# Plachtaa/VALL-E-X

Hardware: AMD Instinct MI355X
Metric: audio-seconds/sec (AR+NAR+Vocos end to end; AR codec-tokens/sec in ar_tokens_per_s), batch32 8s utt (higher is better)
Workload: dtype f32 (cached AR decode step) + f16x2 (operands split into fp16 head + tail = 22 significant bits, tail x tail dropped, fp32 accumulate) for the prefill / NAR projections and full-sequence attention

## Files before the change

vall-e-x_amd/_build.py:

```python
from __future__ import annotations

import os
import subprocess
import sys
from concurrent.futures import ThreadPoolExecutor

HERE = os.path.dirname(os.path.abspath(__file__))
CSRC = os.path.join(HERE, "csrc")
LIB = os.path.join(CSRC, "libvallex_hip.so")
PREFLIGHT = os.path.join(CSRC, "vx_preflight.bin")
SOURCES = ["gemm_f32.hip", "gemm_f16x2.hip", "gemm_bf16x3.hip", "gemm_bf16x3_dma.hip", "rows.hip", "attn_full.hip", "attn_full_x3.hip", "attn_full_h2.hip", "decode.hip", "beams.hip", "admit.hip", "serve.hip", "serve_sample.hip", "vocos.hip", "encodec.hip", "engine.hip", "weights.hip", "vocoders.hip", "bench_harness.hip"]
HEADERS = ["vx_common.h"]
ENGINE_TUS = ("engine.hip", "beams.hip", "admit.hip", "serve.hip", "serve_sample.hip", "weights.hip", "vocoders.hip", "bench_harness.hip")
ENGINE_HEADERS = ["engine_ctx.h", os.path.join("..", "..", "include", "vallex_hip.h"),
                  os.path.join("..", "..", "include", "vallex_hip_dev.h")]
FLAGS = ["--offload-arch=gfx950", "-O3", "-std=c++17", "-fPIC", "-Wall", "-Wno-unused-result",
         "-mllvm", "-amdgpu-kernarg-preload-count=16"]


def _hipcc() -> str:
    for cand in (os.environ.get("HIPCC"), "/opt/rocm/bin/hipcc", "hipcc"):
        if cand and (os.path.sep not in cand or os.path.exists(cand)):
            return cand
    return "hipcc"


def _digest(paths, extra=()) -> str:
    import hashlib
    h = hashlib.sha256()
# ... 91 lines not shown
```

vall-e-x_amd/csrc/engine.hip:

```cpp
#include "engine_ctx.h"

#include <deque>
#include <memory>

namespace {
thread_local std::string g_create_err;
}

namespace vxe {

const float* W(vx_ctx* c, const std::string& name) {
  auto it = c->w.find(name);
  return it == c->w.end() ? nullptr : it->second.d;
}

static int ring_slot(vx_ctx* c, size_t n, char** slot) {
  PinRing& r = c->ring;
  if (!r.base) FAIL(VX_ESTATE, "the context has no pinned transfer ring");
  const size_t a = (n + 255) & ~(size_t)255;
  if (r.head + a > r.cap) if (int e = xfer_sync(c)) return e;
  *slot = r.base + r.head;
  r.head += a;
  return VX_OK;
}
// ... 424 lines not shown
  a.uniforms_stride = c->cur_batch;
  a.seed_dev = c->seed_dev;
  a.force_eos_at = s ? s->force_eos_at : -1;
  a.commit = commit;
  a.cur_tok = c->cur_tok; a.cur_pos = c->cur_pos; a.ctx_len = c->ctx_len; a.n_gen = c->n_gen; a.active = c->active;
  a.n_active = c->n_active; a.slot_meta = c->slot_meta; a.slot_of = c->slot_of;
  a.text_len = c->text_len; a.gen = c->gen; a.gen_stride = c->gen_stride; a.logits_out = logits_out;
  a.sum_logp = (s && s->best_of > 1) ? c->sum_logp : nullptr;
  a.batch = c->cur_batch;
  if (commit) {
    a.emb_tab = W(c, "ar_audio_embedding.word_embeddings.weight"); a.emb_alpha = W(c, "ar_audio_position.alpha");
    a.pe = c->pe; a.ln_g = c->ar[0].n1_w; a.ln_b = c->ar[0].n1_b; a.emb_h = c->dh; a.emb_xp = c->xp;
    a.wt = c->sb_chain ? 0 : 1;
  }
  return a;
}

void ar_step_launches(vx_ctx* c, const SampleArgs* sa, const ServeSampleArgs* rsa) {
  const int nb = c->cur_batch, NL = c->NL;
  hipStream_t st = c->stream;
  const size_t cache_layer = (size_t)c->mbr * N_HEAD * c->Tmax * D_HEAD;
  if (!sa && !rsa)
    launch_dec_embed_ln_pack(c->cur_tok, c->cur_pos, W(c, "ar_audio_embedding.word_embeddings.weight"),
                             W(c, "ar_audio_position.alpha"), c->pe, c->dh, c->ar[0].n1_w, c->ar[0].n1_b, c->xp, nb, st);
  if (c->sb_chain) {
    float *hr = c->dh, *hw = c->dh2;
    for (int l = 0; l < NL; ++l) {
      const LayerW& L = c->ar[l];
      if (c->sb_qkv) {
        {
// ... 24 lines not shown
      { ProfScope ps(c, 1); LAUNCH(launch_skinny_gemm_sb_combine(L.out_wp, c->p_o, D_MODEL, SK_OUT, c->part_o, c->part_ml, c->nsplit, nb, st)); }
      }
      {
        ProfScope ps(c, 1);
        LAUNCH(launch_skinny16_sb_ln(L.l1_wp, L.l1_b, c->xp4, D_FF, c->p_o, SK_OUT, L.out_b, hr, hw, L.n2_w, L.n2_b, nb, st));
        std::swap(hr, hw);
      }
      { ProfScope ps(c, 1); launch_skinny_gemm(L.l2_wp, c->xp4, c->p_o, D_MODEL, D_FF, SK_L2, st); }
    }
    {
      ProfScope ps(c, 1);
      LAUNCH(launch_skinny_gemm_sb_ln(c->pred_wp, c->p_logits, PRED_NPAD, SK_PRED, c->p_o, SK_L2, c->ar[NL - 1].l2_b, hr, nullptr,
                               W(c, "ar_decoder.norm.weight"), W(c, "ar_decoder.norm.bias"), nb, st));
    }
    if (rsa) LAUNCH(launch_serve_sample(*rsa, st));
    else if (sa) LAUNCH(launch_dec_sample(*sa, st));
    return;
  }
  for (int l = 0; l < NL; ++l) {
    const LayerW& L = c->ar[l];
    {
      ProfScope ps(c, 1);
      if (c->qkv_bal) launch_skinny_qkv_balanced(L.in_wp, c->xp, c->p_qkv, st);
      else launch_skinny_gemm(L.in_wp, c->xp, c->p_qkv, 3 * D_MODEL, D_MODEL, SK_QKV, st, true);
    }
    const bool fused = c->fuse_out && (c->nsplit == 1 || c->split_fused);
    {
      ProfScope ps(c, 0);
      LAUNCH(launch_dec_attn(c->p_qkv, c->qkv_bal ? SK_QKV_BALANCED : SK_QKV, L.in_b, c->kc + l * cache_layer, c->vc + l * cache_layer, c->Tmax, c->slot_meta,
                      c->xp_att, c->part_o, c->part_ml, c->nsplit, nb, fused ? L.out_wh : nullptr, c->p_oh, st));
    }
// ... 2 lines not shown
    } else if (fused) {
      launch_dec_reduce_ln_pack(c->p_oh, N_HEAD, D_MODEL, L.out_b, c->dh, c->dh, L.n2_w, L.n2_b, c->xp, nb, st);
    } else {
      if (c->nsplit > 1) launch_dec_attn_combine(c->part_o, c->part_ml, c->nsplit, c->active, c->xp_att, nb, st);
      { ProfScope ps(c, 1); launch_skinny_gemm(L.out_wp, c->xp_att, c->p_o, D_MODEL, D_MODEL, SK_OUT, st, true); }
      launch_dec_reduce_ln_pack(c->p_o, SK_OUT, D_MODEL, L.out_b, c->dh, c->dh, L.n2_w, L.n2_b, c->xp, nb, st);
    }
    { ProfScope ps(c, 1); launch_skinny16_relu_pack(L.l1_wp, c->xp, L.l1_b, c->xp4, D_FF, D_MODEL, st); }
    { ProfScope ps(c, 1); launch_skinny_gemm(L.l2_wp, c->xp4, c->p_o, D_MODEL, D_FF, SK_L2, st, true); }
    const float* ng = (l + 1 < NL) ? c->ar[l + 1].n1_w : W(c, "ar_decoder.norm.weight");
    const float* nbp = (l + 1 < NL) ? c->ar[l + 1].n1_b : W(c, "ar_decoder.norm.bias");
    launch_dec_reduce_ln_pack(c->p_o, SK_L2, D_MODEL, L.l2_b, c->dh, c->dh, ng, nbp, c->xp, nb, st);
  }
  { ProfScope ps(c, 1); launch_skinny_gemm(c->pred_wp, c->xp, c->p_logits, PRED_NPAD, D_MODEL, SK_PRED, st, true); }
  if (rsa) LAUNCH(launch_serve_sample(*rsa, st));
  else if (sa) LAUNCH(launch_dec_sample(*sa, st));
}

static_assert(SK_QKV == 4, "dec_attn_kernel<*, 4> sums four QKV slabs in its prologue");
static_assert(SK_OUT == 4, "skinny16_sb_kernel<4> / dec_reduce_ln_pack<4> are the instantiated out_proj consumers");
static_assert(SK_L2 == 8 || SK_L2 == 4, "skinny_gemm_sb_kernel<0, 8 | 4> are the instantiated linear2 consumers");
static_assert(SK_PRED == 4 || SK_PRED == 2 || SK_PRED == 1, "dec_sample_kernel<4 | 2 | 1>");

int launch_status(vx_ctx* c) {
  if (!c->launch_fail) return VX_OK;
  const char* what = c->launch_fail;
  c->launch_fail = nullptr;
  FAIL(VX_EINVAL, "kernel configuration not compiled into this library: %s", what);
}

constexpr int GRAPH_STEPS = 4;
// ... 49 lines not shown
    const long steps = std::min<long>(s->uniforms_steps, c->gen_stride + 1);
    if (steps * nb > c->uniforms_cap) FAIL(VX_EINVAL, "too many uniforms (%ld steps)", steps);
    std::vector<float> u((size_t)steps * nb);
    for (long t = 0; t < steps; ++t)
      for (int i = 0; i < nb; ++i) u[t * nb + i] = s->uniforms[t * ub + (long)r0 * beams + i];
    H2D(c->d_uniforms, u.data(), u.size() * sizeof(float));
    SYNC();
  }
  H2D(c->seed_dev, &seed, sizeof seed);
  SampleArgs sa = make_sample_args(c, s, 1, nullptr);
  std::vector<int> act(nb);
  bool any = true, raised = false;
  auto first_sample = [&]() -> int {
    int flag = 0;
    HIPCHK(hipMemsetAsync(c->sum_logp, 0, MB * sizeof(float), c->stream));
    LAUNCH(launch_dec_sample(sa, c->stream));
    if (int e = launch_status(c)) return e;
    D2H(act.data(), c->active, nb * sizeof(int));
    if (range_guarded(c) && !direct_f32) D2H(&flag, c->range_flag, sizeof(int));
    SYNC();
    raised = flag != 0;
    any = std::any_of(act.begin(), act.end(), [](int v) { return v != 0; });
    return VX_OK;
  };
  if (int e = first_sample()) return e;
  if (!direct_f32) fb_outcome(c, raised, c->fb_prefill_raises, c->sticky_prefill_f32, c->sticky_prefill_age);
  if (raised) {
    HIPCHK(hipMemsetAsync(c->range_flag, 0, sizeof(int), c->stream));
    ++c->st_fb_prefill; ++c->fb_total;
    if (int e = ensure_f32_buffers(c)) return e;
    {
      F32Scope f32(c);
      if (int e = ar_prefill(c, b, r0, nb_rows, beams)) return e;
      if (int e = first_sample()) return e;
    }
  }
  char sig[160];
  snprintf(sig, sizeof sig, "b%d ns%d c%d%d%d k%d t%a u%d f%d l%d", nb, c->nsplit, (int)c->sb_chain, (int)c->sb_qkv, (int)c->split_fused, sa.top_k, sa.temperature,
           sa.uniforms != nullptr, sa.force_eos_at, sa.sum_logp != nullptr);
  const int sync_every = s->sync_every > 0 ? s->sync_every : 8;
  const int hard_cap = s->force_eos_at >= 0 ? std::min(c->gen_stride + 2, s->force_eos_at) : c->gen_stride + 2;
  int steps = 0;
  const int gs = (c->graph_multi && sync_every % GRAPH_STEPS == 0) ? GRAPH_STEPS : 1;
  while (any && steps < hard_cap) {
    const int n = (steps % gs == 0 && steps + gs <= hard_cap) ? gs : 1;
    if (int e = ar_step_run(c, &sa, sig, n)) return e;
    steps += n;
    if (steps % sync_every == 0) {
      D2H(act.data(), c->active, nb * sizeof(int));
      SYNC();
      any = std::any_of(act.begin(), act.end(), [](int v) { return v != 0; });
    }
  }
  n_gen.resize(nb);
// ... 234 lines not shown
    adm[drow[i]] = 1;
  }
  const long o_tab = mb.add(tab), o_adm = mb.add(adm), o_saved = mb.add(saved);
  UniformCols uc;
  if (int e = uniform_cols(c, b, s, drow, crow, mb, uc)) return e;
  if (int e = upload_meta(c)) return e;
  uniform_cols_launch(c, s, uc, mb);
  if (int e = prefill_layers(c, p, mb)) return e;
  launch_admit_rows(mb.dev(o_tab), k, prefill_hsrc(c, p), c->dh2, c->cur_tok, c->cur_pos, c->ctx_len, c->n_gen, c->text_len,
                    c->slot_meta, c->slot_of, c->stream);
  launch_dec_reduce_ln_pack(nullptr, 0, D_MODEL, nullptr, c->dh2, nullptr, W(c, "ar_decoder.norm.weight"),
                            W(c, "ar_decoder.norm.bias"), c->xp_att, nd, c->stream);
  launch_skinny_gemm(c->pred_wp, c->xp_att, c->p_logits, PRED_NPAD, D_MODEL, SK_PRED, c->stream);
  int* sv = c->imeta + o_saved;
  launch_admit_mask(0, mb.dev(o_adm), sv, nd, c->active, c->slot_meta, c->slot_of, c->n_active, c->stream);
  LAUNCH(launch_dec_sample(sa, c->stream));
  launch_admit_mask(1, mb.dev(o_adm), sv, nd, c->active, c->slot_meta, c->slot_of, c->n_active, c->stream);
  return launch_status(c);
}

int infer_continuous(vx_ctx* c, const vx_batch* b, const vx_sampling* s, vx_row_done_fn on_row, void* user, int64_t* out_codes,
                     int32_t out_stride, int32_t* out_lens) {
  const int B = b->batch, nd = std::min(c->mbr, B);
  hipEvent_t e0 = c->ev_t[0], e1 = c->ev_t[1], e2 = c->ev_t[2];
  HIPCHK(hipEventRecord(e0, c->stream));
  std::vector<int> occ(nd, -1), done_by(nd, 0), act(nd, 0), ng(nd, 0), slot_of(nd);
  std::vector<std::vector<int>> rowgen(B);
  std::vector<int> pend;
  int next = 0;
  long steps = 0;
  const int first_cap = s->force_eos_at >= 0 ? std::min(c->gen_stride, s->force_eos_at) : c->gen_stride;
// ... 3 lines not shown
  };
  SampleArgs sa{};
  auto round = [&](const std::vector<int>& drow, const std::vector<int>& crow) -> int {
    const bool first = occ[0] < 0 && next == 0;
    bool raised = false;
    auto attempt = [&](bool read_flag) -> int {
      if (first) {
        if (int e = ar_prefill(c, b, 0, nd)) return e;
        sa = make_sample_args(c, s, 1, nullptr);
        sa.uniforms = c->d_uniforms;
        MetaBuilder mb(c);
        UniformCols uc;
        if (int e = uniform_cols(c, b, s, drow, crow, mb, uc)) return e;
        if (int e = upload_meta(c)) return e;
        uniform_cols_launch(c, s, uc, mb);
        LAUNCH(launch_dec_sample(sa, c->stream));
        if (int e = launch_status(c)) return e;
        D2H(slot_of.data(), c->slot_of, nd * sizeof(int));
      } else if (int e = admit_rows(c, b, s, sa, drow, crow, slot_of)) return e;
      int flag = 0;
      D2H(act.data(), c->active, nd * sizeof(int));
      D2H(ng.data(), c->n_gen, nd * sizeof(int));
      if (read_flag) D2H(&flag, c->range_flag, sizeof(int));
      SYNC();
      raised = flag != 0;
      return VX_OK;
    };
    const bool direct_f32 = fb_direct(c, c->sticky_prefill_f32, c->sticky_prefill_age);
    if (direct_f32) {
      ++c->st_fb_prefill; ++c->fb_total;
      if (int e = ensure_f32_buffers(c)) return e;
// ... 42 lines not shown
        o[0] = codes0[(size_t)i * c->gen_stride + t];
        for (int st = 0; st < N_Q - 1; ++st) o[st + 1] = oc[(size_t)st * sumT + off + t];
      }
      off += T[i];
      if (on_row) on_row(user, r, o0, T[i]);
    }
    return VX_OK;
  };

  {
    std::vector<int> first(nd);
    for (int i = 0; i < nd; ++i) first[i] = i;
    if (int e = round(first, first)) return e;
  }
  char sig[160];
  snprintf(sig, sizeof sig, "b%d ns%d c%d%d%d k%d t%a u%d f%d l%d", nd, c->nsplit, (int)c->sb_chain, (int)c->sb_qkv, (int)c->split_fused, sa.top_k,
           sa.temperature, sa.uniforms != nullptr, sa.force_eos_at, sa.sum_logp != nullptr);
  const int sync_every = s->sync_every > 0 ? s->sync_every : 8;
  const int gs = (c->graph_multi && sync_every % GRAPH_STEPS == 0) ? GRAPH_STEPS : 1;
  for (;;) {
    std::vector<int> freed;
    for (int d = 0; d < nd; ++d) {
      if (occ[d] < 0 || act[d]) continue;
      const int r = occ[d];
      if (ng[d] > out_stride) FAIL(VX_EINVAL, "out_stride %d too small for %d frames", out_stride, ng[d]);
      rowgen[r].assign(ng[d], 0);
      if (ng[d]) D2H(rowgen[r].data(), c->gen + (size_t)d * c->gen_stride, ng[d] * sizeof(int));
      pend.push_back(r);
      occ[d] = -1;
    }
    for (int d = 0; d < nd; ++d) if (occ[d] < 0) freed.push_back(d);
    if (next < B && !freed.empty()) {
// ... 704 lines not shown
  for (int d = 0; d < v->nd; ++d) v->slot_of[d] = d;
  if (!c->row_smp) {
    if (int e = dev_alloc(c, &c->row_smp, 4 * MB)) { delete v; return e; }
  }
  if (int e = serve_setup(c, v->nd)) { delete v; return e; }
  const SampleArgs sa = make_sample_args(c, &v->s, 1, nullptr);
  ServeSampleArgs& r = v->rsa;
  r.partial = sa.partial; r.splitk = sa.splitk; r.npad = sa.npad;
  r.row_smp = c->row_smp;
  r.uniforms = c->d_uniforms; r.uniforms_stride = sa.uniforms_stride;
  r.cur_tok = sa.cur_tok; r.cur_pos = sa.cur_pos; r.ctx_len = sa.ctx_len; r.n_gen = sa.n_gen; r.active = sa.active;
  r.n_active = sa.n_active; r.text_len = sa.text_len; r.slot_meta = sa.slot_meta; r.slot_of = sa.slot_of;
  r.gen = sa.gen; r.gen_stride = sa.gen_stride; r.sum_logp = c->sum_logp; r.batch = sa.batch;
  r.emb_tab = sa.emb_tab; r.emb_alpha = sa.emb_alpha; r.pe = sa.pe; r.ln_g = sa.ln_g; r.ln_b = sa.ln_b; r.emb_h = sa.emb_h;
  r.emb_xp = sa.emb_xp; r.wt = sa.wt;
  char sig[160];
  snprintf(sig, sizeof sig, "b%d ns%d c%d%d%d serve-rows u1 l1", v->nd, c->nsplit, (int)c->sb_chain, (int)c->sb_qkv, (int)c->split_fused);
  v->sig = sig;
  c->serve = v;
  *out = v;
  return VX_OK;
}

int vx_serve_submit(vx_serve* v, const vx_batch* b, const vx_request* req, int64_t* ids_out) {
  if (!v || !req) return VX_EINVAL;
  return serve_submit(v, b, req, nullptr, ids_out);
}

int vx_serve_submit_ex(vx_serve* v, const vx_batch* b, const vx_request* req, const vx_request_sampling* smp, int64_t* ids_out) {
  if (!v || !req) return VX_EINVAL;
  return serve_submit(v, b, req, smp, ids_out);
}
// ... 102 lines not shown
```

vall-e-x_amd/csrc/engine_ctx.h:

```cpp
#pragma once

#include <math.h>
#include <stdio.h>
#include <stdlib.h>
#include <string.h>

#include <algorithm>
#include <array>
#include <map>
#include <string>
#include <thread>
#include <vector>

#include "../../include/vallex_hip.h"
#include "vx_common.h"

using namespace vx;

namespace vxe {

struct Tensor {
  float* d = nullptr;
  std::vector<int64_t> shape;
  size_t n = 0;
// ... 69 lines not shown
  unsigned short* fa3 = nullptr;
  unsigned short* pred_w3[N_Q - 1] = {};
  float *fx = nullptr, *fxn = nullptr, *fqkv = nullptr, *fatt = nullptr, *fffn = nullptr, *fyemb = nullptr,
        *flogits = nullptr;
  int* imeta = nullptr;
  long imeta_cap = 0;
  std::vector<int> hmeta;

  float *kc = nullptr, *vc = nullptr;
  float *dh = nullptr, *dh2 = nullptr, *xp = nullptr, *xp_att = nullptr, *xp4 = nullptr;
  bool sb_qkv = false;
  int sb_qkv_rows = 4, sb_qkv_nsplit = 0;
  bool sb_chain = false;
  bool sb_fuse = true;
  bool qkv_bal = true;
  float* qk_new = nullptr;
  float *p_qkv = nullptr, *p_o = nullptr, *p_oh = nullptr, *p_logits = nullptr, *part_o = nullptr, *part_ml = nullptr;
  std::map<const unsigned short*, int> w_shift;
  bool nar_trim = true;
  bool balance_rows = true;
  bool fuse_out = true;
  int fuse_split = 1;
  bool split_fused = false;
  float *d_logits = nullptr, *d_uniforms = nullptr, *sum_logp = nullptr;
  long uniforms_cap = 0;
  int *cur_tok = nullptr, *cur_pos = nullptr, *ctx_len = nullptr, *n_gen = nullptr, *active = nullptr,
      *text_len = nullptr, *gen = nullptr, *force_tok = nullptr, *n_active = nullptr, *slot_meta = nullptr, *slot_of = nullptr;
  int gen_stride = 0;
  int cur_batch = 0;
  int nsplit = 1;
// ... 153 lines not shown
                           int* row_smp, hipStream_t s);
void launch_serve_cancel(unsigned rows, int nrows, int* active, int* slot_meta, const int* slot_of, int* n_active, hipStream_t s);

struct ServeSampleArgs {
  const float* partial; int splitk; int npad;
  const int* row_smp;
  const float* uniforms; int uniforms_stride;
  int* cur_tok; int* cur_pos; int* ctx_len; int* n_gen; int* active; int* n_active; const int* text_len;
  int* slot_meta; const int* slot_of;
  int* gen; int gen_stride;
  float* sum_logp;
  int batch;
  const float* emb_tab; const float* emb_alpha; const float* pe; const float* ln_g; const float* ln_b;
  float* emb_h; float* emb_xp;
  int wt;
};
bool launch_serve_sample(const ServeSampleArgs& a, hipStream_t s);

struct F32Scope {
  vx_ctx* c;
  int gm;
  bool ax;
  explicit F32Scope(vx_ctx* c_) : c(c_), gm(c_->gemm_mode), ax(c_->attn_x3) { c->gemm_mode = 2; c->attn_x3 = false; }
  ~F32Scope() { c->gemm_mode = gm; c->attn_x3 = ax; }
};

}
```

vall-e-x_amd/csrc/serve_sample.hip:

```cpp
#include "engine_ctx.h"

namespace vxe {
namespace {

constexpr int SPL = 17;

__device__ __forceinline__ void store_wt(float* p, const f32x4& v, bool wt) {
  if (wt) asm volatile("global_store_dwordx4 %0, %1, off sc1" :: "v"(p), "v"(v) : "memory");
  else *reinterpret_cast<f32x4*>(p) = v;
}

__device__ __forceinline__ float sum64f(float v) {
  int x = __builtin_bit_cast(int, v);
  v += __builtin_bit_cast(float, __builtin_amdgcn_update_dpp(0, x, 0xB1, 0xF, 0xF, true));
  x = __builtin_bit_cast(int, v);
  v += __builtin_bit_cast(float, __builtin_amdgcn_update_dpp(0, x, 0x4E, 0xF, 0xF, true));
  x = __builtin_bit_cast(int, v);
  v += __builtin_bit_cast(float, __builtin_amdgcn_update_dpp(0, x, 0x141, 0xF, 0xF, true));
  x = __builtin_bit_cast(int, v);
  v += __builtin_bit_cast(float, __builtin_amdgcn_update_dpp(0, x, 0x140, 0xF, 0xF, true));
  x = __builtin_bit_cast(int, v);
  v += __builtin_bit_cast(float, __builtin_amdgcn_update_dpp(0, x, 0x142, 0xA, 0xF, false));
  x = __builtin_bit_cast(int, v);
  v += __builtin_bit_cast(float, __builtin_amdgcn_update_dpp(0, x, 0x143, 0xC, 0xF, false));
// ... 45 lines not shown
    for (int e = 0; e < 4; ++e) { const float d = v[i][e] - mean; q += d * d; }
  const float rstd = 1.0f / sqrtf(sum64f(q) * (1.0f / D_MODEL) + LN_EPS);
#pragma unroll
  for (int i = 0; i < 4; ++i) {
    const int c4 = lane + 64 * i;
    f32x4 o;
#pragma unroll
    for (int e = 0; e < 4; ++e) o[e] = (v[i][e] - mean) * rstd * gg[i][e] + be[i][e];
    store_wt(xp + (((long)(c4 >> 1) * 64) + b + 32 * (c4 & 1)) * 4, o, wt);
  }
}

template <int SK>
__global__ __launch_bounds__(64) void serve_sample_kernel(ServeSampleArgs a) {
  __shared__ float lg[64 * SPL];
  const int b = blockIdx.x, lane = threadIdx.x;
  if (a.active[b] == 0) return;
  const int ngen = a.n_gen[b], pos = a.cur_pos[b], ctx = a.ctx_len[b], tlen = a.text_len[b], slot = a.slot_of[b];
  const int4 smp = *reinterpret_cast<const int4*>(a.row_smp + 4 * b);
  const int top_k = smp.x, force_eos_at = smp.z;
  const float temperature = __builtin_bit_cast(float, smp.y);
  {
    float pp[SPL][SK];
#pragma unroll
    for (int i = 0; i < SPL; ++i) {
      const int n = lane + 64 * i, nc = n < AR_LOGITS ? n : AR_LOGITS - 1;
#pragma unroll
      for (int ks = 0; ks < SK; ++ks) pp[i][ks] = a.partial[((long)ks * MB + b) * a.npad + nc];
    }
#pragma unroll
    for (int i = 0; i < SPL; ++i) {
      const int n = lane + 64 * i;
      float t = pp[i][0];
      if (SK == 2) t = t + pp[i][1];
      if (SK == 4) t = ((t + pp[i][1]) + pp[i][2]) + pp[i][3];
      if (n >= AR_LOGITS) t = -INFINITY;
      lg[n] = t;
    }
  }
  __syncthreads();

  const float u = a.uniforms[(long)ngen * a.uniforms_stride + b];
  f32x4 pe4[4], gg[4], be[4];
  float alpha = 0.f;
// ... 3 lines not shown
    for (int i = 0; i < 4; ++i) {
      const int c = (lane + 64 * i) * 4;
      pe4[i] = *reinterpret_cast<const f32x4*>(a.pe + (long)(pos + 1) * D_MODEL + c);
      gg[i] = *reinterpret_cast<const f32x4*>(a.ln_g + c);
      be[i] = *reinterpret_cast<const f32x4*>(a.ln_b + c);
    }
  }

  float v[SPL];
#pragma unroll
  for (int j = 0; j < SPL; ++j) v[j] = lg[lane * SPL + j];
  if (temperature != 1.0f) {
#pragma unroll
    for (int j = 0; j < SPL; ++j) v[j] = v[j] / temperature;
  }
  float mx = -INFINITY;
#pragma unroll
  for (int j = 0; j < SPL; ++j) mx = fmaxf(mx, v[j]);
  mx = max64f(mx);

  if (top_k > 0 && top_k < AR_LOGITS) {
    float thr = mx;
    for (int it = 1; it < top_k && thr != -INFINITY; ++it) {
      float cur = -INFINITY;
#pragma unroll
      for (int j = 0; j < SPL; ++j) if (v[j] < thr) cur = fmaxf(cur, v[j]);
      thr = max64f(cur);
    }
    int cnt = 0;
#pragma unroll
    for (int j = 0; j < SPL; ++j) cnt += (v[j] >= thr);
    if (sum64i(cnt) != top_k) {
      float prev = INFINITY;
      int count = 0;
      thr = mx;
      while (true) {
        float cur = -INFINITY;
#pragma unroll
        for (int j = 0; j < SPL; ++j) if (v[j] < prev) cur = fmaxf(cur, v[j]);
        cur = max64f(cur);
        int c2 = 0;
#pragma unroll
        for (int j = 0; j < SPL; ++j) c2 += (v[j] == cur);
        count += sum64i(c2);
        thr = cur;
        if (count >= top_k || cur == -INFINITY) break;
        prev = cur;
      }
    }
#pragma unroll
    for (int j = 0; j < SPL; ++j) if (v[j] < thr) v[j] = -INFINITY;
  }
  float e[SPL], loc = 0.f;
#pragma unroll
  for (int j = 0; j < SPL; ++j) { e[j] = expf(v[j] - mx); loc += e[j]; }
  float incl = loc;
#pragma unroll
  for (int o = 1; o < 64; o <<= 1) {
    const float t = __shfl_up(incl, o, 64);
    if (lane >= o) incl += t;
  }
  const float total = __builtin_bit_cast(float, __builtin_amdgcn_readlane(__builtin_bit_cast(int, incl), 63));
  const float thresh = u * total;
  float c = incl - loc;
  int cand = 0x7fffffff, lastnz = -1;
#pragma unroll
  for (int j = 0; j < SPL; ++j) {
    if (e[j] > 0.f) {
      c += e[j];
      lastnz = lane * SPL + j;
      if (c > thresh && cand == 0x7fffffff) cand = lane * SPL + j;
    }
  }
  cand = minmax64i<false>(cand);
  const int last_all = minmax64i<true>(lastnz);
  int tok = cand == 0x7fffffff ? last_all : cand;
  if ((unsigned)tok > (unsigned)EOS_ID) tok = EOS_ID;

  if (tok / SPL == lane) {
    float vt = 0.f;
#pragma unroll
    for (int j = 0; j < SPL; ++j) if (tok - lane * SPL == j) vt = v[j];
    a.sum_logp[b] += (vt - mx) - logf(total);
  }

  if (force_eos_at >= 0 && ngen >= force_eos_at) tok = EOS_ID;
  const bool stop = tok == EOS_ID || (1 + ngen) > 16 * tlen || ngen >= a.gen_stride;
  if (lane == 0) {
    if (stop) {
      a.active[b] = 0;
// ... 36 lines not shown
```

vall-e-x_amd/csrc/weights.hip:

```cpp
#include "engine_ctx.h"

namespace {

int need(vx_ctx* c, const std::string& name, std::initializer_list<int64_t> shape) {
  auto it = c->w.find(name);
  if (it == c->w.end()) FAIL(VX_ENOTFOUND, "missing tensor '%s'", name.c_str());
  if (it->second.shape != std::vector<int64_t>(shape)) FAIL(VX_EINVAL, "tensor '%s' has the wrong shape", name.c_str());
  return VX_OK;
}

int pack(vx_ctx* c, const float* Wt, int N, int K, int Npad, float** out) {
  if (int e = dev_alloc(c, out, (size_t)Npad * K, false)) return e;
  launch_pack_weight(Wt, N, K, *out, Npad, c->stream);
  return VX_OK;
}

}

extern "C" {

int vx_load_tensor(vx_ctx* c, const char* name, const float* data, const int64_t* shape, int32_t ndim) {
  if (!c) return VX_EINVAL;
  if (!name || !data || !shape || ndim < 0 || ndim > 4) FAIL(VX_EINVAL, "bad tensor argument");
  if (c->finalized) FAIL(VX_ESTATE, "weights already finalized");
// ... 96 lines not shown
  if (range_guarded(c) && (e = ensure_f32_buffers(c))) return e;
  if ((e = dev_alloc(c, &c->fyemb, (size_t)M * d))) return e;
  if ((e = dev_alloc(c, &c->flogits, (size_t)((long)c->mbr * c->cfg.max_new + 128) * AUDIO_VOCAB))) return e;
  c->imeta_cap = std::max(M * 24, (long)c->cfg.max_batch * c->cfg.max_new * 12) + 65536;
  if ((e = dev_alloc(c, &c->imeta, (size_t)c->imeta_cap))) return e;
  const size_t cache = (size_t)NL * c->mbr * N_HEAD * c->Tmax * D_HEAD;
  if ((e = dev_alloc(c, &c->kc, cache, true))) return e;
  if ((e = dev_alloc(c, &c->vc, cache, true))) return e;
  if ((e = dev_alloc(c, &c->dh, (size_t)MB * d))) return e;
  if ((e = dev_alloc(c, &c->dh2, (size_t)MB * d))) return e;
  if (const char* ev = getenv("VX_SB_FUSE")) c->sb_fuse = !(ev[0] == '0');
  if ((e = dev_alloc(c, &c->xp, (size_t)MB * d))) return e;
  if ((e = dev_alloc(c, &c->xp_att, (size_t)MB * d))) return e;
  if ((e = dev_alloc(c, &c->xp4, (size_t)2 * MB * f))) return e;
  if (const char* ev = getenv("VX_QKV_BALANCED")) c->qkv_bal = !(ev[0] == '0');
  static_assert(SK_QKV_BAL_Q == 8 && SK_QKV_BAL_KV == SK_QKV, "skinny_qkv_bal_kernel writes 8 q slabs and SK_QKV k / v slabs into p_qkv");
  if ((e = dev_alloc(c, &c->p_qkv, (size_t)std::max(SK_QKV, SK_QKV_BAL_Q) * MB * 3 * d))) return e;
  if ((e = dev_alloc(c, &c->p_o, (size_t)std::max(SK_OUT, SK_L2) * MB * d))) return e;
  if ((e = dev_alloc(c, &c->p_oh, (size_t)4 * N_HEAD * MB * d))) return e;
  if (const char* ev = getenv("VX_FUSE_OUT")) c->fuse_out = !(ev[0] == '0');
  if (c->Tmax < DEC_ATTN_TILE) c->fuse_out = false;
  if (const char* ev = getenv("VX_BALANCE_ROWS")) c->balance_rows = !(ev[0] == '0');
  if (const char* ev = getenv("VX_NAR_TRIM")) c->nar_trim = ev[0] == '1';
  if (const char* ev = getenv("VX_GRAPH_MULTI")) c->graph_multi = !(ev[0] == '0');
  if (const char* ev = getenv("VX_SB_QKV")) c->sb_qkv_rows = atoi(ev);
  if (const char* ev = getenv("VX_SB_QKV_NSPLIT")) c->sb_qkv_nsplit = atoi(ev);
  if (const char* ev = getenv("VX_FUSE_SPLIT")) c->fuse_split = atoi(ev);
  if (const char* ev = getenv("VX_ATT_NSPLIT")) c->att_nsplit_force = std::max(0, std::min(16, atoi(ev)));
  if ((e = dev_alloc(c, &c->p_logits, (size_t)SK_PRED * MB * PRED_NPAD))) return e;
  if ((e = dev_alloc(c, &c->part_o, (size_t)MB * N_HEAD * 16 * D_HEAD))) return e;
// ... 392 lines not shown
```

Baseline: 378.4.

## Add fast single-pass top-k selection for AR sampling kernels

Adds a new sampling kernel and a shared selection header. It finds the top-k candidates in one pass, using a per-lane-max threshold plus ballot compaction into LDS, instead of the iterative max-below-threshold loop that costs one wave reduction per k. It also uses DPP for the prefix scan and skips the last-nonzero reduction unless it is needed. The decode, serve and admit paths route to this kernel by default, and the old loop stays as a fallback when more than 64 candidates or ties are present. Tie-breaking and floating-point equivalence are risks, and the extra LDS use could change occupancy.

Result: no change. 380.5 (median of 6 runs) (+0.6%).

```diff
diff --git a/vall-e-x_amd/_build.py b/vall-e-x_amd/_build.py
--- a/vall-e-x_amd/_build.py
+++ b/vall-e-x_amd/_build.py
@@ -9,10 +9,10 @@
 CSRC = os.path.join(HERE, "csrc")
 LIB = os.path.join(CSRC, "libvallex_hip.so")
 PREFLIGHT = os.path.join(CSRC, "vx_preflight.bin")
-SOURCES = ["gemm_f32.hip", "gemm_f16x2.hip", "gemm_bf16x3.hip", "gemm_bf16x3_dma.hip", "rows.hip", "attn_full.hip", "attn_full_x3.hip", "attn_full_h2.hip", "decode.hip", "beams.hip", "admit.hip", "serve.hip", "serve_sample.hip", "vocos.hip", "encodec.hip", "engine.hip", "weights.hip", "vocoders.hip", "bench_harness.hip"]
+SOURCES = ["gemm_f32.hip", "gemm_f16x2.hip", "gemm_bf16x3.hip", "gemm_bf16x3_dma.hip", "rows.hip", "attn_full.hip", "attn_full_x3.hip", "attn_full_h2.hip", "decode.hip", "beams.hip", "admit.hip", "serve.hip", "serve_sample.hip", "sample_fast.hip", "vocos.hip", "encodec.hip", "engine.hip", "weights.hip", "vocoders.hip", "bench_harness.hip"]
 HEADERS = ["vx_common.h"]
-ENGINE_TUS = ("engine.hip", "beams.hip", "admit.hip", "serve.hip", "serve_sample.hip", "weights.hip", "vocoders.hip", "bench_harness.hip")
-ENGINE_HEADERS = ["engine_ctx.h", os.path.join("..", "..", "include", "vallex_hip.h"),
+ENGINE_TUS = ("engine.hip", "beams.hip", "admit.hip", "serve.hip", "serve_sample.hip", "sample_fast.hip", "weights.hip", "vocoders.hip", "bench_harness.hip")
+ENGINE_HEADERS = ["engine_ctx.h", "sample_select.h", os.path.join("..", "..", "include", "vallex_hip.h"),
                   os.path.join("..", "..", "include", "vallex_hip_dev.h")]
 FLAGS = ["--offload-arch=gfx950", "-O3", "-std=c++17", "-fPIC", "-Wall", "-Wno-unused-result",
          "-mllvm", "-amdgpu-kernarg-preload-count=16"]
diff --git a/vall-e-x_amd/csrc/engine.hip b/vall-e-x_amd/csrc/engine.hip
--- a/vall-e-x_amd/csrc/engine.hip
+++ b/vall-e-x_amd/csrc/engine.hip
@@ -462,6 +462,13 @@
     a.wt = c->sb_chain ? 0 : 1;
   }
   return a;
+}
+
+static bool sample_fast_applies(const vx_ctx* c, const SampleArgs& sa) {
+  return c->sample_fast && sa.commit && !sa.logits_out && sa.top_k >= 1 && sa.top_k <= 64;
+}
+static bool launch_sample(vx_ctx* c, const SampleArgs& sa, hipStream_t st) {
+  return sample_fast_applies(c, sa) ? launch_dec_sample_fast(sa, st) : launch_dec_sample(sa, st);
 }
 
 void ar_step_launches(vx_ctx* c, const SampleArgs* sa, const ServeSampleArgs* rsa) {
@@ -516,7 +523,7 @@
                                W(c, "ar_decoder.norm.weight"), W(c, "ar_decoder.norm.bias"), nb, st));
     }
     if (rsa) LAUNCH(launch_serve_sample(*rsa, st));
-    else if (sa) LAUNCH(launch_dec_sample(*sa, st));
+    else if (sa) LAUNCH(launch_sample(c, *sa, st));
     return;
   }
   for (int l = 0; l < NL; ++l) {
@@ -549,7 +556,7 @@
   }
   { ProfScope ps(c, 1); launch_skinny_gemm(c->pred_wp, c->xp, c->p_logits, PRED_NPAD, D_MODEL, SK_PRED, st, true); }
   if (rsa) LAUNCH(launch_serve_sample(*rsa, st));
-  else if (sa) LAUNCH(launch_dec_sample(*sa, st));
+  else if (sa) LAUNCH(launch_sample(c, *sa, st));
 }
 
 static_assert(SK_QKV == 4, "dec_attn_kernel<*, 4> sums four QKV slabs in its prologue");
@@ -629,7 +636,7 @@
   auto first_sample = [&]() -> int {
     int flag = 0;
     HIPCHK(hipMemsetAsync(c->sum_logp, 0, MB * sizeof(float), c->stream));
-    LAUNCH(launch_dec_sample(sa, c->stream));
+    LAUNCH(launch_sample(c, sa, c->stream));
     if (int e = launch_status(c)) return e;
     D2H(act.data(), c->active, nb * sizeof(int));
     if (range_guarded(c) && !direct_f32) D2H(&flag, c->range_flag, sizeof(int));
@@ -651,8 +658,8 @@
     }
   }
   char sig[160];
-  snprintf(sig, sizeof sig, "b%d ns%d c%d%d%d k%d t%a u%d f%d l%d", nb, c->nsplit, (int)c->sb_chain, (int)c->sb_qkv, (int)c->split_fused, sa.top_k, sa.temperature,
-           sa.uniforms != nullptr, sa.force_eos_at, sa.sum_logp != nullptr);
+  snprintf(sig, sizeof sig, "b%d ns%d c%d%d%d k%d t%a u%d f%d l%d s%d", nb, c->nsplit, (int)c->sb_chain, (int)c->sb_qkv, (int)c->split_fused, sa.top_k, sa.temperature,
+           sa.uniforms != nullptr, sa.force_eos_at, sa.sum_logp != nullptr, (int)sample_fast_applies(c, sa));
   const int sync_every = s->sync_every > 0 ? s->sync_every : 8;
   const int hard_cap = s->force_eos_at >= 0 ? std::min(c->gen_stride + 2, s->force_eos_at) : c->gen_stride + 2;
   int steps = 0;
@@ -917,7 +924,7 @@
   launch_skinny_gemm(c->pred_wp, c->xp_att, c->p_logits, PRED_NPAD, D_MODEL, SK_PRED, c->stream);
   int* sv = c->imeta + o_saved;
   launch_admit_mask(0, mb.dev(o_adm), sv, nd, c->active, c->slot_meta, c->slot_of, c->n_active, c->stream);
-  LAUNCH(launch_dec_sample(sa, c->stream));
+  LAUNCH(launch_sample(c, sa, c->stream));
   launch_admit_mask(1, mb.dev(o_adm), sv, nd, c->active, c->slot_meta, c->slot_of, c->n_active, c->stream);
   return launch_status(c);
 }
@@ -951,7 +958,7 @@
         if (int e = uniform_cols(c, b, s, drow, crow, mb, uc)) return e;
         if (int e = upload_meta(c)) return e;
         uniform_cols_launch(c, s, uc, mb);
-        LAUNCH(launch_dec_sample(sa, c->stream));
+        LAUNCH(launch_sample(c, sa, c->stream));
         if (int e = launch_status(c)) return e;
         D2H(slot_of.data(), c->slot_of, nd * sizeof(int));
       } else if (int e = admit_rows(c, b, s, sa, drow, crow, slot_of)) return e;
@@ -1024,8 +1031,8 @@
     if (int e = round(first, first)) return e;
   }
   char sig[160];
-  snprintf(sig, sizeof sig, "b%d ns%d c%d%d%d k%d t%a u%d f%d l%d", nd, c->nsplit, (int)c->sb_chain, (int)c->sb_qkv, (int)c->split_fused, sa.top_k,
-           sa.temperature, sa.uniforms != nullptr, sa.force_eos_at, sa.sum_logp != nullptr);
+  snprintf(sig, sizeof sig, "b%d ns%d c%d%d%d k%d t%a u%d f%d l%d s%d", nd, c->nsplit, (int)c->sb_chain, (int)c->sb_qkv, (int)c->split_fused, sa.top_k,
+           sa.temperature, sa.uniforms != nullptr, sa.force_eos_at, sa.sum_logp != nullptr, (int)sample_fast_applies(c, sa));
   const int sync_every = s->sync_every > 0 ? s->sync_every : 8;
   const int gs = (c->graph_multi && sync_every % GRAPH_STEPS == 0) ? GRAPH_STEPS : 1;
   for (;;) {
@@ -1760,8 +1767,9 @@
   r.gen = sa.gen; r.gen_stride = sa.gen_stride; r.sum_logp = c->sum_logp; r.batch = sa.batch;
   r.emb_tab = sa.emb_tab; r.emb_alpha = sa.emb_alpha; r.pe = sa.pe; r.ln_g = sa.ln_g; r.ln_b = sa.ln_b; r.emb_h = sa.emb_h;
   r.emb_xp = sa.emb_xp; r.wt = sa.wt;
+  r.fast = c->sample_fast ? 1 : 0;
   char sig[160];
-  snprintf(sig, sizeof sig, "b%d ns%d c%d%d%d serve-rows u1 l1", v->nd, c->nsplit, (int)c->sb_chain, (int)c->sb_qkv, (int)c->split_fused);
+  snprintf(sig, sizeof sig, "b%d ns%d c%d%d%d serve-rows u1 l1 s%d", v->nd, c->nsplit, (int)c->sb_chain, (int)c->sb_qkv, (int)c->split_fused, r.fast);
   v->sig = sig;
   c->serve = v;
   *out = v;
diff --git a/vall-e-x_amd/csrc/engine_ctx.h b/vall-e-x_amd/csrc/engine_ctx.h
--- a/vall-e-x_amd/csrc/engine_ctx.h
+++ b/vall-e-x_amd/csrc/engine_ctx.h
@@ -107,6 +107,7 @@
   bool sb_chain = false;
   bool sb_fuse = true;
   bool qkv_bal = true;
+  bool sample_fast = true;
   float* qk_new = nullptr;
   float *p_qkv = nullptr, *p_o = nullptr, *p_oh = nullptr, *p_logits = nullptr, *part_o = nullptr, *part_ml = nullptr;
   std::map<const unsigned short*, int> w_shift;
@@ -290,8 +291,10 @@
   const float* emb_tab; const float* emb_alpha; const float* pe; const float* ln_g; const float* ln_b;
   float* emb_h; float* emb_xp;
   int wt;
+  int fast;
 };
 bool launch_serve_sample(const ServeSampleArgs& a, hipStream_t s);
+bool launch_dec_sample_fast(const SampleArgs& a, hipStream_t s);
 
 struct F32Scope {
   vx_ctx* c;
diff --git a/vall-e-x_amd/csrc/sample_fast.hip b/vall-e-x_amd/csrc/sample_fast.hip
--- /dev/null
+++ b/vall-e-x_amd/csrc/sample_fast.hip
@@ -0,0 +1,246 @@
+#include "engine_ctx.h"
+#include "sample_select.h"
+
+namespace vxe {
+namespace {
+
+constexpr int SPL = sel::SPL;
+
+__device__ __forceinline__ void store_wt(float* p, const f32x4& v, bool wt) {
+  if (wt) asm volatile("global_store_dwordx4 %0, %1, off sc1" :: "v"(p), "v"(v) : "memory");
+  else *reinterpret_cast<f32x4*>(p) = v;
+}
+
+__device__ __forceinline__ float sum64f(float v) {
+  int x = __builtin_bit_cast(int, v);
+  v += __builtin_bit_cast(float, __builtin_amdgcn_update_dpp(0, x, 0xB1, 0xF, 0xF, true));
+  x = __builtin_bit_cast(int, v);
+  v += __builtin_bit_cast(float, __builtin_amdgcn_update_dpp(0, x, 0x4E, 0xF, 0xF, true));
+  x = __builtin_bit_cast(int, v);
+  v += __builtin_bit_cast(float, __builtin_amdgcn_update_dpp(0, x, 0x141, 0xF, 0xF, true));
+  x = __builtin_bit_cast(int, v);
+  v += __builtin_bit_cast(float, __builtin_amdgcn_update_dpp(0, x, 0x140, 0xF, 0xF, true));
+  x = __builtin_bit_cast(int, v);
+  v += __builtin_bit_cast(float, __builtin_amdgcn_update_dpp(0, x, 0x142, 0xA, 0xF, false));
+  x = __builtin_bit_cast(int, v);
+  v += __builtin_bit_cast(float, __builtin_amdgcn_update_dpp(0, x, 0x143, 0xC, 0xF, false));
+  return __builtin_bit_cast(float, __builtin_amdgcn_readlane(__builtin_bit_cast(int, v), 63));
+}
+__device__ __forceinline__ float max64f(float x) {
+  int v = __builtin_bit_cast(int, x);
+  x = fmaxf(x, __builtin_bit_cast(float, __builtin_amdgcn_update_dpp(v, v, 0xB1, 0xF, 0xF, false)));
+  v = __builtin_bit_cast(int, x);
+  x = fmaxf(x, __builtin_bit_cast(float, __builtin_amdgcn_update_dpp(v, v, 0x4E, 0xF, 0xF, false)));
+  v = __builtin_bit_cast(int, x);
+  x = fmaxf(x, __builtin_bit_cast(float, __builtin_amdgcn_update_dpp(v, v, 0x141, 0xF, 0xF, false)));
+  v = __builtin_bit_cast(int, x);
+  x = fmaxf(x, __builtin_bit_cast(float, __builtin_amdgcn_update_dpp(v, v, 0x140, 0xF, 0xF, false)));
+  v = __builtin_bit_cast(int, x);
+  x = fmaxf(x, __builtin_bit_cast(float, __builtin_amdgcn_update_dpp(v, v, 0x142, 0xA, 0xF, false)));
+  v = __builtin_bit_cast(int, x);
+  x = fmaxf(x, __builtin_bit_cast(float, __builtin_amdgcn_update_dpp(v, v, 0x143, 0xC, 0xF, false)));
+  return __builtin_bit_cast(float, __builtin_amdgcn_readlane(__builtin_bit_cast(int, x), 63));
+}
+template <bool MAX>
+__device__ __forceinline__ int minmax64i(int v) {
+#define VX_MM(CTRL, RM) { const int t = __builtin_amdgcn_update_dpp(v, v, CTRL, RM, 0xF, false); v = MAX ? max(v, t) : min(v, t); }
+  VX_MM(0xB1, 0xF) VX_MM(0x4E, 0xF) VX_MM(0x141, 0xF) VX_MM(0x140, 0xF) VX_MM(0x142, 0xA) VX_MM(0x143, 0xC)
+#undef VX_MM
+  return __builtin_amdgcn_readlane(v, 63);
+}
+__device__ __forceinline__ int sum64i(int x) {
+  x += __builtin_amdgcn_update_dpp(0, x, 0xB1, 0xF, 0xF, true);
+  x += __builtin_amdgcn_update_dpp(0, x, 0x4E, 0xF, 0xF, true);
+  x += __builtin_amdgcn_update_dpp(0, x, 0x141, 0xF, 0xF, true);
+  x += __builtin_amdgcn_update_dpp(0, x, 0x140, 0xF, 0xF, true);
+  x += __builtin_amdgcn_update_dpp(0, x, 0x142, 0xA, 0xF, false);
+  x += __builtin_amdgcn_update_dpp(0, x, 0x143, 0xC, 0xF, false);
+  return __builtin_amdgcn_readlane(x, 63);
+}
+
+__device__ __forceinline__ void ln_pack(const f32x4 (&v)[4], int b, const f32x4 (&gg)[4], const f32x4 (&be)[4], float* __restrict__ xp,
+                                        bool wt) {
+  const int lane = threadIdx.x;
+  float s = 0.f;
+#pragma unroll
+  for (int i = 0; i < 4; ++i) s += (v[i][0] + v[i][1]) + (v[i][2] + v[i][3]);
+  const float mean = sum64f(s) * (1.0f / D_MODEL);
+  float q = 0.f;
+#pragma unroll
+  for (int i = 0; i < 4; ++i)
+#pragma unroll
+    for (int e = 0; e < 4; ++e) { const float d = v[i][e] - mean; q += d * d; }
+  const float rstd = 1.0f / sqrtf(sum64f(q) * (1.0f / D_MODEL) + LN_EPS);
+#pragma unroll
+  for (int i = 0; i < 4; ++i) {
+    const int c4 = lane + 64 * i;
+    f32x4 o;
+#pragma unroll
+    for (int e = 0; e < 4; ++e) o[e] = (v[i][e] - mean) * rstd * gg[i][e] + be[i][e];
+    store_wt(xp + (((long)(c4 >> 1) * 64) + b + 32 * (c4 & 1)) * 4, o, wt);
+  }
+}
+
+__device__ __forceinline__ unsigned long long splitmix64(unsigned long long x) {
+  x += 0x9E3779B97F4A7C15ull;
+  x = (x ^ (x >> 30)) * 0xBF58476D1CE4E5B9ull;
+  x = (x ^ (x >> 27)) * 0x94D049BB133111EBull;
+  return x ^ (x >> 31);
+}
+
+template <int SK>
+__global__ __launch_bounds__(64) void dec_sample_fast_kernel(SampleArgs a) {
+  __shared__ float lg[64 * SPL];
+  __shared__ sel::Lds sl;
+  const int b = blockIdx.x, lane = threadIdx.x;
+  if (a.active[b] == 0) return;
+  const int ngen = a.n_gen[b], pos = a.cur_pos[b], ctx = a.ctx_len[b], tlen = a.text_len[b], slot = a.slot_of[b];
+  const unsigned long long seed = a.uniforms ? 0ull : a.seed_dev[0];
+  {
+    float pp[SPL][SK];
+#pragma unroll
+    for (int i = 0; i < SPL; ++i) {
+      const int n = lane + 64 * i, nc = n < AR_LOGITS ? n : AR_LOGITS - 1;
+#pragma unroll
+      for (int ks = 0; ks < SK; ++ks) pp[i][ks] = a.partial[((long)ks * MB + b) * a.npad + nc];
+    }
+    sel::lds_init(sl);
+#pragma unroll
+    for (int i = 0; i < SPL; ++i) {
+      const int n = lane + 64 * i;
+      float t = pp[i][0];
+      if (SK == 2) t = t + pp[i][1];
+      if (SK == 4) t = ((t + pp[i][1]) + pp[i][2]) + pp[i][3];
+      if (n >= AR_LOGITS) t = -INFINITY;
+      lg[n] = t;
+    }
+  }
+  __syncthreads();
+
+  float u;
+  if (a.uniforms) u = a.uniforms[(long)ngen * a.uniforms_stride + b];
+  else
+    u = (float)(splitmix64(splitmix64(splitmix64(seed) + (unsigned long long)b) + (unsigned long long)ngen) >> 40) *
+        (1.0f / 16777216.0f);
+  f32x4 pe4[4], gg[4], be[4];
+  float alpha = 0.f;
+  if (a.emb_tab) {
+    alpha = a.emb_alpha[0];
+#pragma unroll
+    for (int i = 0; i < 4; ++i) {
+      const int c = (lane + 64 * i) * 4;
+      pe4[i] = *reinterpret_cast<const f32x4*>(a.pe + (long)(pos + 1) * D_MODEL + c);
+      gg[i] = *reinterpret_cast<const f32x4*>(a.ln_g + c);
+      be[i] = *reinterpret_cast<const f32x4*>(a.ln_b + c);
+    }
+  }
+
+  float v[SPL];
+#pragma unroll
+  for (int j = 0; j < SPL; ++j) v[j] = lg[lane * SPL + j];
+  if (a.temperature != 1.0f) {
+#pragma unroll
+    for (int j = 0; j < SPL; ++j) v[j] = v[j] / a.temperature;
+  }
+  float lmax = -INFINITY;
+#pragma unroll
+  for (int j = 0; j < SPL; ++j) lmax = fmaxf(lmax, v[j]);
+  const float mx = max64f(lmax);
+
+  float e[SPL];
+  if (!sel::topk_numerators(sl, v, lmax, mx, a.top_k, e)) {
+    if (a.top_k > 0 && a.top_k < AR_LOGITS) {
+      float thr = mx;
+      for (int it = 1; it < a.top_k && thr != -INFINITY; ++it) {
+        float cur = -INFINITY;
+#pragma unroll
+        for (int j = 0; j < SPL; ++j) if (v[j] < thr) cur = fmaxf(cur, v[j]);
+        thr = max64f(cur);
+      }
+      int cnt = 0;
+#pragma unroll
+      for (int j = 0; j < SPL; ++j) cnt += (v[j] >= thr);
+      if (sum64i(cnt) != a.top_k) {
+        float prev = INFINITY;
+        int count = 0;
+        thr = mx;
+        while (true) {
+          float cur = -INFINITY;
+#pragma unroll
+          for (int j = 0; j < SPL; ++j) if (v[j] < prev) cur = fmaxf(cur, v[j]);
+          cur = max64f(cur);
+          int c2 = 0;
+#pragma unroll
+          for (int j = 0; j < SPL; ++j) c2 += (v[j] == cur);
+          count += sum64i(c2);
+          thr = cur;
+          if (count >= a.top_k || cur == -INFINITY) break;
+          prev = cur;
+        }
+      }
+#pragma unroll
+      for (int j = 0; j < SPL; ++j) if (v[j] < thr) v[j] = -INFINITY;
+    }
+#pragma unroll
+    for (int j = 0; j < SPL; ++j) e[j] = expf(v[j] - mx);
+  }
+  float loc = 0.f;
+#pragma unroll
+  for (int j = 0; j < SPL; ++j) loc += e[j];
+  const float incl = sel::scan64f(loc);
+  const float total = __builtin_bit_cast(float, __builtin_amdgcn_readlane(__builtin_bit_cast(int, incl), 63));
+  const float thresh = u * total;
+  const int cand = minmax64i<false>(sel::cdf_first(e, incl - loc, thresh));
+  int last_all = -1;
+  if (cand == 0x7fffffff) last_all = minmax64i<true>(sel::cdf_last(e));
+  int tok = cand == 0x7fffffff ? last_all : cand;
+  if ((unsigned)tok > (unsigned)EOS_ID) tok = EOS_ID;
+
+  if (a.sum_logp && tok / SPL == lane) {
+    float vt = 0.f;
+#pragma unroll
+    for (int j = 0; j < SPL; ++j) if (tok - lane * SPL == j) vt = v[j];
+    a.sum_logp[b] += (vt - mx) - logf(total);
+  }
+
+  if (a.force_eos_at >= 0 && ngen >= a.force_eos_at) tok = EOS_ID;
+  const bool stop = tok == EOS_ID || (1 + ngen) > 16 * tlen || ngen >= a.gen_stride;
+  if (lane == 0) {
+    if (stop) {
+      a.active[b] = 0;
+      a.slot_meta[4 * slot + 2] = 0;
+      if (a.n_active) atomicSub(a.n_active, 1);
+    } else {
+      a.gen[(long)b * a.gen_stride + ngen] = tok;
+      a.n_gen[b] = ngen + 1;
+      a.cur_tok[b] = tok;
+      a.cur_pos[b] = pos + 1;
+      a.ctx_len[b] = ctx + 1;
+      a.slot_meta[4 * slot + 1] = ctx + 1;
+    }
+  }
+  if (stop || !a.emb_tab) return;
+  f32x4 hv[4];
+#pragma unroll
+  for (int i = 0; i < 4; ++i) {
+    const int cc = (lane + 64 * i) * 4;
+    hv[i] = *reinterpret_cast<const f32x4*>(a.emb_tab + (long)tok * D_MODEL + cc);
+#pragma unroll
+    for (int q = 0; q < 4; ++q) hv[i][q] = __fadd_rn(hv[i][q], __fmul_rn(alpha, pe4[i][q]));
+    store_wt(a.emb_h + (long)b * D_MODEL + cc, hv[i], a.wt != 0);
+  }
+  ln_pack(hv, b, gg, be, a.emb_xp, a.wt != 0);
+}
+
+}
+
+bool launch_dec_sample_fast(const SampleArgs& a, hipStream_t s) {
+  if (!a.commit || a.logits_out || a.top_k < 1 || a.top_k > sel::MAX_K) return launch_dec_sample(a, s);
+  if (a.splitk == 4) hipLaunchKernelGGL(dec_sample_fast_kernel<4>, dim3(a.batch), dim3(64), 0, s, a);
+  else if (a.splitk == 2) hipLaunchKernelGGL(dec_sample_fast_kernel<2>, dim3(a.batch), dim3(64), 0, s, a);
+  else if (a.splitk == 1) hipLaunchKernelGGL(dec_sample_fast_kernel<1>, dim3(a.batch), dim3(64), 0, s, a);
+  else return false;
+  return true;
+}
+
+}
diff --git a/vall-e-x_amd/csrc/sample_select.h b/vall-e-x_amd/csrc/sample_select.h
--- /dev/null
+++ b/vall-e-x_amd/csrc/sample_select.h
@@ -0,0 +1,145 @@
+#pragma once
+#include "vx_common.h"
+
+namespace vxe {
+namespace sel {
+
+using vx::f32x4;
+
+constexpr int SPL = 17;
+constexpr int MAX_K = 64;
+constexpr int QUAD_K = 12;
+
+struct __attribute__((aligned(16))) Lds {
+  float img[64 * SPL];
+  float lm[64];
+  float cv[64 * SPL];
+  int ci[64 * SPL];
+};
+
+__device__ __forceinline__ float min64f(float x) {
+  int k = __builtin_bit_cast(int, x);
+  k ^= (k >> 31) & 0x7fffffff;
+#define VX_SEL_MIN(CTRL, RM) k = min(k, __builtin_amdgcn_update_dpp(k, k, CTRL, RM, 0xF, false));
+  VX_SEL_MIN(0xB1, 0xF) VX_SEL_MIN(0x4E, 0xF) VX_SEL_MIN(0x141, 0xF) VX_SEL_MIN(0x140, 0xF) VX_SEL_MIN(0x142, 0xA) VX_SEL_MIN(0x143, 0xC)
+#undef VX_SEL_MIN
+  k = __builtin_amdgcn_readlane(k, 63);
+  k ^= (k >> 31) & 0x7fffffff;
+  return __builtin_bit_cast(float, k);
+}
+__device__ __forceinline__ float quad_max(float x) {
+  int v = __builtin_bit_cast(int, x);
+  x = fmaxf(x, __builtin_bit_cast(float, __builtin_amdgcn_update_dpp(v, v, 0xB1, 0xF, 0xF, false)));
+  v = __builtin_bit_cast(int, x);
+  return fmaxf(x, __builtin_bit_cast(float, __builtin_amdgcn_update_dpp(v, v, 0x4E, 0xF, 0xF, false)));
+}
+
+__device__ __forceinline__ void lds_init(Lds& s) {
+  const int lane = threadIdx.x;
+  const f32x4 z = {0.f, 0.f, 0.f, 0.f};
+#pragma unroll
+  for (int i = 0; i < (64 * SPL / 4 + 63) / 64; ++i) {
+    const int q = lane + 64 * i;
+    if (q < 64 * SPL / 4) *reinterpret_cast<f32x4*>(&s.img[4 * q]) = z;
+  }
+  s.cv[lane] = -INFINITY;
+}
+
+__device__ __forceinline__ int above4(const f32x4& q, float x) { return (q[0] > x) + (q[1] > x) + (q[2] > x) + (q[3] > x); }
+
+__device__ __forceinline__ bool topk_numerators(Lds& s, const float (&v)[SPL], float lmax, float mx, int top_k, float (&e)[SPL]) {
+  const int lane = threadIdx.x;
+  if (top_k < 1 || top_k > MAX_K) return false;
+
+  float p;
+  if (top_k <= QUAD_K) {
+    const float g = quad_max(lmax);
+    int above = 0;
+#pragma unroll
+    for (int i = 0; i < 16; ++i)
+      above += __builtin_bit_cast(float, __builtin_amdgcn_readlane(__builtin_bit_cast(int, g), 4 * i)) > g;
+    p = min64f(above < top_k ? g : INFINITY);
+  } else {
+    s.lm[lane] = lmax;
+    __syncthreads();
+    f32x4 q[16];
+#pragma unroll
+    for (int i = 0; i < 16; ++i) q[i] = *reinterpret_cast<const f32x4*>(&s.lm[4 * i]);
+    __builtin_amdgcn_sched_barrier(0);
+    int above = 0;
+#pragma unroll
+    for (int i = 0; i < 16; ++i) above += above4(q[i], lmax);
+    p = min64f(above < top_k ? lmax : INFINITY);
+  }
+  if (!(p > -INFINITY)) return false;
+
+  int n = 0;
+#pragma unroll
+  for (int j = 0; j < SPL; ++j) {
+    const bool c = !(v[j] < p);
+    const unsigned long long m = __builtin_amdgcn_ballot_w64(c);
+    const int slot = (int)__builtin_amdgcn_mbcnt_hi((unsigned)(m >> 32), __builtin_amdgcn_mbcnt_lo((unsigned)m, (unsigned)n));
+    if (c) { s.cv[slot] = v[j]; s.ci[slot] = lane * SPL + j; }
+    n += __builtin_popcountll(m);
+  }
+  if (n > MAX_K) return false;
+  __syncthreads();
+  const float c = s.cv[lane];
+  const int ci = s.ci[lane];
+  f32x4 h[4];
+#pragma unroll
+  for (int i = 0; i < 4; ++i) h[i] = *reinterpret_cast<const f32x4*>(&s.cv[4 * i]);
+  __builtin_amdgcn_sched_barrier(0);
+  if (__builtin_amdgcn_ballot_w64(!(c < INFINITY)) != 0) return false;
+
+  int above_c = 0;
+#pragma unroll
+  for (int i = 0; i < 4; ++i) above_c += above4(h[i], c);
+  for (int i = 16; i < n; i += 4) above_c += above4(*reinterpret_cast<const f32x4*>(&s.cv[i]), c);
+  const float thr = min64f((lane < n && above_c < top_k) ? c : INFINITY);
+
+  if (lane < n && c >= thr) s.img[ci] = expf(c - mx);
+  __syncthreads();
+#pragma unroll
+  for (int j = 0; j < SPL; ++j) e[j] = s.img[lane * SPL + j];
+  return true;
+}
+
+__device__ __forceinline__ int cdf_first(const float (&e)[SPL], float c, float thresh) {
+  int first = 0;
+  bool open = true;
+#pragma unroll
+  for (int j = 0; j < SPL; ++j) {
+    c += e[j];
+    open = open && !(e[j] > 0.f && c > thresh);
+    first += open;
+  }
+  return first < SPL ? (int)threadIdx.x * SPL + first : 0x7fffffff;
+}
+__device__ __forceinline__ int cdf_last(const float (&e)[SPL]) {
+  int last = -1;
+#pragma unroll
+  for (int j = 0; j < SPL; ++j) last = e[j] > 0.f ? j : last;
+  return last < 0 ? -1 : (int)threadIdx.x * SPL + last;
+}
+
+__device__ __forceinline__ float scan64f(float x) {
+  const int lane = threadIdx.x;
+#pragma unroll
+  for (int o = 1; o < 64; o <<= 1) {
+    float t;
+    if (o <= 4) {
+      int k = __builtin_bit_cast(int, x);
+#pragma unroll
+      for (int i = 0; i < o; ++i) k = __builtin_amdgcn_update_dpp(k, k, 0x138, 0xF, 0xF, false);
+      t = __builtin_bit_cast(float, k);
+    } else {
+      t = __shfl_up(x, o, 64);
+    }
+    if (lane >= o) x += t;
+  }
+  return x;
+}
+
+}
+}
diff --git a/vall-e-x_amd/csrc/serve_sample.hip b/vall-e-x_amd/csrc/serve_sample.hip
--- a/vall-e-x_amd/csrc/serve_sample.hip
+++ b/vall-e-x_amd/csrc/serve_sample.hip
@@ -1,9 +1,10 @@
 #include "engine_ctx.h"
+#include "sample_select.h"
 
 namespace vxe {
 namespace {
 
-constexpr int SPL = 17;
+constexpr int SPL = sel::SPL;
 
 __device__ __forceinline__ void store_wt(float* p, const f32x4& v, bool wt) {
   if (wt) asm volatile("global_store_dwordx4 %0, %1, off sc1" :: "v"(p), "v"(v) : "memory");
@@ -83,6 +84,7 @@
 template <int SK>
 __global__ __launch_bounds__(64) void serve_sample_kernel(ServeSampleArgs a) {
   __shared__ float lg[64 * SPL];
+  __shared__ sel::Lds sl;
   const int b = blockIdx.x, lane = threadIdx.x;
   if (a.active[b] == 0) return;
   const int ngen = a.n_gen[b], pos = a.cur_pos[b], ctx = a.ctx_len[b], tlen = a.text_len[b], slot = a.slot_of[b];
@@ -97,6 +99,7 @@
 #pragma unroll
       for (int ks = 0; ks < SK; ++ks) pp[i][ks] = a.partial[((long)ks * MB + b) * a.npad + nc];
     }
+    sel::lds_init(sl);
 #pragma unroll
     for (int i = 0; i < SPL; ++i) {
       const int n = lane + 64 * i;
@@ -130,66 +133,57 @@
 #pragma unroll
     for (int j = 0; j < SPL; ++j) v[j] = v[j] / temperature;
   }
-  float mx = -INFINITY;
-#pragma unroll
-  for (int j = 0; j < SPL; ++j) mx = fmaxf(mx, v[j]);
-  mx = max64f(mx);
-
-  if (top_k > 0 && top_k < AR_LOGITS) {
-    float thr = mx;
-    for (int it = 1; it < top_k && thr != -INFINITY; ++it) {
-      float cur = -INFINITY;
-#pragma unroll
-      for (int j = 0; j < SPL; ++j) if (v[j] < thr) cur = fmaxf(cur, v[j]);
-      thr = max64f(cur);
-    }
-    int cnt = 0;
-#pragma unroll
-    for (int j = 0; j < SPL; ++j) cnt += (v[j] >= thr);
-    if (sum64i(cnt) != top_k) {
-      float prev = INFINITY;
-      int count = 0;
-      thr = mx;
-      while (true) {
+  float lmax = -INFINITY;
+#pragma unroll
+  for (int j = 0; j < SPL; ++j) lmax = fmaxf(lmax, v[j]);
+  const float mx = max64f(lmax);
+
+  float e[SPL];
+  if (!(a.fast && sel::topk_numerators(sl, v, lmax, mx, top_k, e))) {
+    if (top_k > 0 && top_k < AR_LOGITS) {
+      float thr = mx;
+      for (int it = 1; it < top_k && thr != -INFINITY; ++it) {
         float cur = -INFINITY;
 #pragma unroll
-        for (int j = 0; j < SPL; ++j) if (v[j] < prev) cur = fmaxf(cur, v[j]);
-        cur = max64f(cur);
-        int c2 = 0;
-#pragma unroll
-        for (int j = 0; j < SPL; ++j) c2 += (v[j] == cur);
-        count += sum64i(c2);
-        thr = cur;
-        if (count >= top_k || cur == -INFINITY) break;
-        prev = cur;
+        for (int j = 0; j < SPL; ++j) if (v[j] < thr) cur = fmaxf(cur, v[j]);
+        thr = max64f(cur);
       }
-    }
-#pragma unroll
-    for (int j = 0; j < SPL; ++j) if (v[j] < thr) v[j] = -INFINITY;
-  }
-  float e[SPL], loc = 0.f;
-#pragma unroll
-  for (int j = 0; j < SPL; ++j) { e[j] = expf(v[j] - mx); loc += e[j]; }
-  float incl = loc;
-#pragma unroll
-  for (int o = 1; o < 64; o <<= 1) {
-    const float t = __shfl_up(incl, o, 64);
-    if (lane >= o) incl += t;
-  }
+      int cnt = 0;
+#pragma unroll
+      for (int j = 0; j < SPL; ++j) cnt += (v[j] >= thr);
+      if (sum64i(cnt) != top_k) {
+        float prev = INFINITY;
+        int count = 0;
+        thr = mx;
+        while (true) {
+          float cur = -INFINITY;
+#pragma unroll
+          for (int j = 0; j < SPL; ++j) if (v[j] < prev) cur = fmaxf(cur, v[j]);
+          cur = max64f(cur);
+          int c2 = 0;
+#pragma unroll
+          for (int j = 0; j < SPL; ++j) c2 += (v[j] == cur);
+          count += sum64i(c2);
+          thr = cur;
+          if (count >= top_k || cur == -INFINITY) break;
+          prev = cur;
+        }
+      }
+#pragma unroll
+      for (int j = 0; j < SPL; ++j) if (v[j] < thr) v[j] = -INFINITY;
+    }
+#pragma unroll
+    for (int j = 0; j < SPL; ++j) e[j] = expf(v[j] - mx);
+  }
+  float loc = 0.f;
+#pragma unroll
+  for (int j = 0; j < SPL; ++j) loc += e[j];
+  const float incl = sel::scan64f(loc);
   const float total = __builtin_bit_cast(float, __builtin_amdgcn_readlane(__builtin_bit_cast(int, incl), 63));
   const float thresh = u * total;
-  float c = incl - loc;
-  int cand = 0x7fffffff, lastnz = -1;
-#pragma unroll
-  for (int j = 0; j < SPL; ++j) {
-    if (e[j] > 0.f) {
-      c += e[j];
-      lastnz = lane * SPL + j;
-      if (c > thresh && cand == 0x7fffffff) cand = lane * SPL + j;
-    }
-  }
-  cand = minmax64i<false>(cand);
-  const int last_all = minmax64i<true>(lastnz);
+  const int cand = minmax64i<false>(sel::cdf_first(e, incl - loc, thresh));
+  int last_all = -1;
+  if (cand == 0x7fffffff) last_all = minmax64i<true>(sel::cdf_last(e));
   int tok = cand == 0x7fffffff ? last_all : cand;
   if ((unsigned)tok > (unsigned)EOS_ID) tok = EOS_ID;
 
diff --git a/vall-e-x_amd/csrc/weights.hip b/vall-e-x_amd/csrc/weights.hip
--- a/vall-e-x_amd/csrc/weights.hip
+++ b/vall-e-x_amd/csrc/weights.hip
@@ -134,6 +134,7 @@
   if ((e = dev_alloc(c, &c->xp_att, (size_t)MB * d))) return e;
   if ((e = dev_alloc(c, &c->xp4, (size_t)2 * MB * f))) return e;
   if (const char* ev = getenv("VX_QKV_BALANCED")) c->qkv_bal = !(ev[0] == '0');
+  if (const char* ev = getenv("VX_SAMPLE_FAST")) c->sample_fast = !(ev[0] == '0');
   static_assert(SK_QKV_BAL_Q == 8 && SK_QKV_BAL_KV == SK_QKV, "skinny_qkv_bal_kernel writes 8 q slabs and SK_QKV k / v slabs into p_qkv");
   if ((e = dev_alloc(c, &c->p_qkv, (size_t)std::max(SK_QKV, SK_QKV_BAL_Q) * MB * 3 * d))) return e;
   if ((e = dev_alloc(c, &c->p_o, (size_t)std::max(SK_OUT, SK_L2) * MB * d))) return e;
```
